# Nikhil-AI-Labs/image-super-resolution-2

Measured on AMD Instinct MI355X. Metric: output MPix/s at x4 SR (256->1024), higher is better.
Workload: dtype bf16 (bf16 MFMA operands, fp32 accumulate, fp32 activations in HBM); 1 GPU; FreqFusion x4 full 3-expert forward (HAT-L + DAT + NAFNet-SR + fusion stack), one 256x256 LR tile -> 1024x1024 per step per GPU (BASELINE configs[1]); seeded synthetic weights (172.3 M params), 1/f-noise tiles; tile=256, parallelism=tile-sharded x1, weights RCCL-broadcast once (0.0 ms), no per-tile collectives, launch=hipGraph replay, tiles_in_flight=2

## Files before the change

image-super-resolution-2_amd/csrc/token_linear.hip:

```cpp
#include "ff_common.h"


struct TokenLinParams {
  const float* x; float* out;
  const float* gamma; const float* beta;
  const __bf16* w;
  const float* bias;
  const float* res; const float* res2; const float* rs2;
  float* xn; int ldxn;
  float* stats; int st_lo, st_hi; float st_eps;
  const float* x2; int ldx2; const float* cm; const float* gw1t; const float* gb1; const float* gw2; float gb2;
  long long M;
  int ldx, ldo, ldr, ldr2, K, N, NT, act;
  float eps;
  int wpi;
};

#define TL_TR 36

#ifndef TL_GELU_SIG
#define TL_GELU_SIG 1
#endif
#define TL_KERNEL token_linear_kernel
#define TL_IMAGES 0
#define TL_OUT16 0
#include "token_linear_kernel.inc"
#undef TL_KERNEL
#undef TL_IMAGES
#define TL_KERNEL token_linear_images_kernel
#define TL_IMAGES 1
#include "token_linear_kernel.inc"
#undef TL_KERNEL
#undef TL_IMAGES
#undef TL_OUT16
#define TL_KERNEL token_linear_rows16_kernel
#define TL_IMAGES 0
#define TL_OUT16 1
#include "token_linear_kernel.inc"
#undef TL_KERNEL
#undef TL_IMAGES
#undef TL_OUT16


extern "C" int ff_token_linear(const float* x, int ldx, float* out, int ldo, long long M, int K, int kpad, int N, int n_tiles,
                               const float* gamma, const float* beta, float eps, const void* w_tiles,
                               const float* bias_padded, int act, const float* res, int ldr, const float* res2, int ldr2,
                               const float* res2_scale, float* xn_out, int ldxn, float* stats_out, int stat_lo, int stat_hi,
                               float stat_eps, int nterms, void* stream) {
  FF_CHECK_ARG(nterms == 1 || nterms == 3, "ff_token_linear: nterms must be 1 (plain bf16) or 3 (split bf16)");
  FF_CHECK_ARG(x && out && w_tiles, "ff_token_linear: null pointer");
  FF_CHECK_ARG(M > 0 && K > 0 && K <= 192 && K % 4 == 0 && N > 0 && n_tiles * 32 >= N, "ff_token_linear: needs K <= 192 (K %% 4 == 0), n_tiles*32 >= N");
  FF_CHECK_ARG(kpad == 64 || kpad == 128 || kpad == 192, "ff_token_linear: kpad must be 64, 128 or 192");
  FF_CHECK_ARG(kpad >= K, "ff_token_linear: kpad < K");
  FF_CHECK_ARG(ldx >= K && ldx % 4 == 0 && ldo >= N && (((uintptr_t)x) & 15) == 0, "ff_token_linear: x rows must be 16-byte aligned");
  FF_CHECK_ARG((gamma == nullptr) == (beta == nullptr), "ff_token_linear: gamma/beta come together");
  FF_CHECK_ARG((((uintptr_t)w_tiles) & 15) == 0 && (!gamma || ((((uintptr_t)gamma) & 15) == 0 && (((uintptr_t)beta) & 15) == 0)), "ff_token_linear: weights / gamma / beta must be 16-byte aligned");
  FF_CHECK_ARG(!res || ldr >= N, "ff_token_linear: ldr too small");
  FF_CHECK_ARG(!res2 || (ldr2 >= N && res2_scale), "ff_token_linear: res2 needs ldr2 >= N and a scale vector");
  FF_CHECK_ARG(!xn_out || (gamma && ldxn >= K && ldxn % 4 == 0 && (((uintptr_t)xn_out) & 15) == 0), "ff_token_linear: xn_out needs LayerNorm parameters and 16-byte aligned rows");
  TokenLinParams p;
  p.x = x; p.out = out; p.gamma = gamma; p.beta = beta; p.w = (const __bf16*)w_tiles; p.bias = bias_padded;
  p.res = res; p.res2 = res2; p.rs2 = res2_scale; p.xn = xn_out; p.ldxn = ldxn; p.M = M; p.ldx = ldx; p.ldo = ldo; p.ldr = ldr; p.ldr2 = ldr2;
  p.K = K; p.N = N; p.NT = n_tiles; p.act = act; p.eps = eps;
  FF_CHECK_ARG(!stats_out || (stat_lo >= 0 && stat_hi > stat_lo && stat_hi <= N && (((uintptr_t)stats_out) & 7) == 0), "ff_token_linear: bad statistics range");
  p.stats = stats_out; p.st_lo = stat_lo; p.st_hi = stat_hi; p.st_eps = stat_eps;
  p.x2 = nullptr; p.ldx2 = 0; p.cm = nullptr; p.gw1t = nullptr; p.gb1 = nullptr; p.gw2 = nullptr; p.gb2 = 0.f; p.wpi = 0;
  const bool vec4 = (N % 4 == 0) && (ldo % 4 == 0) && ((((uintptr_t)out) & 15) == 0) && (!res || (ldr % 4 == 0 && (((uintptr_t)res) & 15) == 0)) &&
           (!res2 || (ldr2 % 4 == 0 && (((uintptr_t)res2) & 15) == 0 && (((uintptr_t)res2_scale) & 15) == 0));
  const int ks = kpad / 16;
  const size_t lds = (size_t)2 * 2 * 32 * (2 * ks + 1) * 16 + (size_t)8 * 32 * TL_TR * 4 + (size_t)8 * 32 * FF_XS_ROW * 4 + (size_t)n_tiles * 32 * 4;
  FF_CHECK_ARG(lds <= 160 * 1024, "ff_token_linear: N too large for the LDS image");
  FF_CHECK_ARG(act == ACT_NONE || act == ACT_GELU, "ff_token_linear: act must be none or gelu");
  const long long nblk = (M + 255) / 256;
  FF_CHECK_ARG(nblk < (1LL << 31), "ff_token_linear: grid too large");
#define TL_LAUNCH(A, KSV, V4, NTM)                                                                                          \
  do {                                                                                                                      \
    static ff_device_once once;                                                                                             \
    if (!ff_raise_lds(once, "ff_token_linear", 160 * 1024, FF_LDS_SAY_ERR, &token_linear_kernel<A, KSV, V4, false, NTM>)) return FF_ERR_LAUNCH; \
    hipLaunchKernelGGL((token_linear_kernel<A, KSV, V4, false, NTM>), dim3((unsigned)nblk), dim3(512), lds, (hipStream_t)stream, p); \
  } while (0)
#define TL_LAUNCH_NT(A, KSV, V4) do { if (nterms == 3) TL_LAUNCH(A, KSV, V4, 3); else TL_LAUNCH(A, KSV, V4, 1); } while (0)
#define TL_LAUNCH_KS(A, V4) do { if (ks == 4) TL_LAUNCH_NT(A, 4, V4); else if (ks == 8) TL_LAUNCH_NT(A, 8, V4); else TL_LAUNCH_NT(A, 12, V4); } while (0)
  if (act == ACT_GELU) { if (vec4) TL_LAUNCH_KS(ACT_GELU, true); else TL_LAUNCH_KS(ACT_GELU, false); }
  else { if (vec4) TL_LAUNCH_KS(ACT_NONE, true); else TL_LAUNCH_KS(ACT_NONE, false); }
#undef TL_LAUNCH_KS
#undef TL_LAUNCH_NT
#undef TL_LAUNCH
  FF_LAUNCH_CHECK("ff_token_linear");
  return FF_OK;
}

extern "C" int ff_token_linear_rows16(const float* x, int ldx, void* out16, int ldo, long long M, int K, int kpad, int N, int n_tiles,
                                      const float* gamma, const float* beta, float eps, const void* w_tiles, const float* bias_padded,
                                      const float* col_scale, int act, const float* res, int ldr, const float* res2, int ldr2,
                                      const float* res2_scale, float* xn_out, int ldxn, float* stats_out, int stat_lo, int stat_hi,
                                      float stat_eps, int nterms, void* stream) {
  FF_CHECK_ARG(nterms == 1 && act == ACT_NONE && !res && !res2 && !res2_scale && !xn_out && !stats_out,
               "ff_token_linear_rows16: plain bf16 (nterms == 1), no activation, no res / res2 / xn_out / stats_out (got nterms=%d act=%d)", nterms, act);
  FF_CHECK_ARG(x && out16 && w_tiles && col_scale, "ff_token_linear_rows16: null pointer");
  FF_CHECK_ARG(M > 0 && K > 0 && K <= 192 && K % 4 == 0 && N > 0 && N % 4 == 0 && n_tiles * 32 >= N, "ff_token_linear_rows16: needs K <= 192, K and N multiples of 4, n_tiles*32 >= N");
  FF_CHECK_ARG(kpad == 64 || kpad == 128 || kpad == 192, "ff_token_linear_rows16: kpad must be 64, 128 or 192");
  FF_CHECK_ARG(kpad >= K, "ff_token_linear_rows16: kpad < K");
  FF_CHECK_ARG(ldx >= K && ldx % 4 == 0 && (((uintptr_t)x) & 15) == 0, "ff_token_linear_rows16: x rows must be 16-byte aligned");
  FF_CHECK_ARG(ldo >= N && ldo % 4 == 0 && (((uintptr_t)out16) & 7) == 0, "ff_token_linear_rows16: out rows must be 8-byte aligned (pitch in bf16 elements, a multiple of 4)");
  FF_CHECK_ARG((gamma == nullptr) == (beta == nullptr), "ff_token_linear_rows16: gamma/beta come together");
  FF_CHECK_ARG(((((uintptr_t)w_tiles) | ((uintptr_t)col_scale)) & 15) == 0 && (!gamma || ((((uintptr_t)gamma) & 15) == 0 && (((uintptr_t)beta) & 15) == 0)), "ff_token_linear_rows16: weights / col_scale / gamma / beta must be 16-byte aligned");
  TokenLinParams p;
  p.x = x; p.out = reinterpret_cast<float*>(out16); p.gamma = gamma; p.beta = beta; p.w = (const __bf16*)w_tiles; p.bias = bias_padded;
  p.res = nullptr; p.res2 = nullptr; p.rs2 = col_scale; p.xn = nullptr; p.ldxn = 0; p.M = M; p.ldx = ldx; p.ldo = ldo; p.ldr = 0; p.ldr2 = 0;
  p.K = K; p.N = N; p.NT = n_tiles; p.act = ACT_NONE; p.eps = eps;
  p.stats = nullptr; p.st_lo = 0; p.st_hi = 0; p.st_eps = 0.f;
  p.x2 = nullptr; p.ldx2 = 0; p.cm = nullptr; p.gw1t = nullptr; p.gb1 = nullptr; p.gw2 = nullptr; p.gb2 = 0.f; p.wpi = 0;
  const int ks = kpad / 16;
  const size_t lds = (size_t)2 * 2 * 32 * (2 * ks + 1) * 16 + (size_t)8 * 32 * TL_TR * 4 + (size_t)8 * 32 * FF_XS_ROW * 4 + (size_t)2 * n_tiles * 32 * 4;
  FF_CHECK_ARG(lds <= 160 * 1024, "ff_token_linear_rows16: N too large for the LDS image");
  const long long nblk = (M + 255) / 256;
  FF_CHECK_ARG(nblk < (1LL << 31), "ff_token_linear_rows16: grid too large");
#define TL_LAUNCH16(KSV)                                                                                                    \
  do {                                                                                                                      \
    static ff_device_once once;                                                                                             \
    if (!ff_raise_lds(once, "ff_token_linear_rows16", 160 * 1024, FF_LDS_SAY_ERR, &token_linear_rows16_kernel<ACT_NONE, KSV, true, false, 1>)) return FF_ERR_LAUNCH; \
    hipLaunchKernelGGL((token_linear_rows16_kernel<ACT_NONE, KSV, true, false, 1>), dim3((unsigned)nblk), dim3(512), lds, (hipStream_t)stream, p); \
  } while (0)
  if (ks == 4) TL_LAUNCH16(4); else if (ks == 8) TL_LAUNCH16(8); else TL_LAUNCH16(12);
#undef TL_LAUNCH16
  FF_LAUNCH_CHECK("ff_token_linear_rows16");
  return FF_OK;
}

static int token_linear_gated_launch(const char* who, const float* x, int ldx, const float* x2, int ldx2, const float* cm, int B, long long rows_per_image,
                                     const float* gw1t, const float* gb1, const float* gw2, float gb2, float* out, int ldo, long long M, int K, int N,
                                     int n_tiles, const void* w_tiles, const float* bias_padded, const float* res, int ldr, int nterms, void* stream) {
  FF_CHECK_ARG(nterms == 1 || nterms == 3, "%s: nterms must be 1 or 3", who);
  FF_CHECK_ARG(x && x2 && cm && gb1 && gw2 && out && w_tiles, "%s: null pointer", who);
  FF_CHECK_ARG(M > 0 && K > 0 && K <= 192 && K % 4 == 0 && N > 0 && N % 4 == 0 && n_tiles * 32 >= N, "%s: needs K <= 192, K and N multiples of 4", who);
  FF_CHECK_ARG(ldx >= K && ldx % 4 == 0 && ldx2 >= K && ldx2 % 4 == 0 && ldo >= N && ldo % 4 == 0 && (!res || (ldr >= N && ldr % 4 == 0)), "%s: rows must be 16-byte aligned", who);
  FF_CHECK_ARG(((((uintptr_t)x) | ((uintptr_t)x2) | ((uintptr_t)cm) | ((uintptr_t)out) | ((uintptr_t)w_tiles) | ((uintptr_t)res)) & 15) == 0, "%s: 16-byte alignment", who);
  const long long wpi = B ? rows_per_image / 256 : 0, nblk = B ? wpi : (M + 255) / 256;
  FF_CHECK_ARG(nblk < (1LL << 31), "%s: grid too large", who);
  TokenLinParams p{};
  p.x = x; p.out = out; p.w = (const __bf16*)w_tiles; p.bias = bias_padded; p.res = res; p.M = M; p.ldx = ldx; p.ldo = ldo; p.ldr = ldr;
  p.K = K; p.N = N; p.NT = n_tiles; p.act = ACT_NONE;
  p.x2 = x2; p.ldx2 = ldx2; p.cm = cm; p.gw1t = gw1t; p.gb1 = gb1; p.gw2 = gw2; p.gb2 = gb2; p.wpi = (int)wpi;
  const size_t lds = (size_t)2 * 2 * 32 * 25 * 16 + (size_t)8 * 32 * TL_TR * 4 + (size_t)8 * 32 * FF_XS_ROW * 4 + (size_t)n_tiles * 32 * 4;
  FF_CHECK_ARG(lds <= 160 * 1024, "%s: N too large for the LDS image", who);
  static ff_device_once once[2];
  if (!(!B ? ff_raise_lds(once[0], who, 160 * 1024, FF_LDS_SAY_ERR, &token_linear_kernel<ACT_NONE, 12, true, true, 3>, &token_linear_kernel<ACT_NONE, 12, true, true, 1>)
           : ff_raise_lds(once[1], who, 160 * 1024, FF_LDS_SAY_ERR, &token_linear_images_kernel<ACT_NONE, 12, true, true, 3>, &token_linear_images_kernel<ACT_NONE, 12, true, true, 1>)))
    return FF_ERR_LAUNCH;
  const dim3 grid((unsigned)nblk, B ? (unsigned)B : 1u);
  if (!B) {
    if (nterms == 3) hipLaunchKernelGGL((token_linear_kernel<ACT_NONE, 12, true, true, 3>), grid, dim3(512), lds, (hipStream_t)stream, p);
    else hipLaunchKernelGGL((token_linear_kernel<ACT_NONE, 12, true, true, 1>), grid, dim3(512), lds, (hipStream_t)stream, p);
  } else {
    if (nterms == 3) hipLaunchKernelGGL((token_linear_images_kernel<ACT_NONE, 12, true, true, 3>), grid, dim3(512), lds, (hipStream_t)stream, p);
    else hipLaunchKernelGGL((token_linear_images_kernel<ACT_NONE, 12, true, true, 1>), grid, dim3(512), lds, (hipStream_t)stream, p);
  }
  FF_LAUNCH_CHECK(who);
  return FF_OK;
}

extern "C" int ff_token_linear_gated(const float* x, int ldx, const float* x2, int ldx2, const float* cm, const float* gw1t,
                                     const float* gb1, const float* gw2, float gb2, float* out, int ldo, long long M, int K, int N,
                                     int n_tiles, const void* w_tiles, const float* bias_padded, const float* res, int ldr, int nterms,
                                     void* stream) {
  return token_linear_gated_launch("ff_token_linear_gated", x, ldx, x2, ldx2, cm, 0, 0, gw1t, gb1, gw2, gb2, out, ldo, M, K, N, n_tiles, w_tiles, bias_padded, res, ldr, nterms, stream);
}

extern "C" int ff_token_linear_gated_images(const float* x, int ldx, const float* x2, int ldx2, const float* cm, int B, long long rows_per_image,
                                            const float* gb1, const float* gw2, float gb2, float* out, int ldo, long long M, int K, int N,
                                            int n_tiles, const void* w_tiles, const float* bias_padded, const float* res, int ldr, int nterms,
                                            void* stream) {
  FF_CHECK_ARG(B > 0 && B <= 65535 && rows_per_image > 0 && rows_per_image % 256 == 0 && M == (long long)B * rows_per_image,
               "ff_token_linear_gated_images: rows_per_image must be a positive multiple of 256 and M == B * rows_per_image (1 <= B <= 65535; got B=%d rows_per_image=%lld M=%lld)",
               B, rows_per_image, M);
  return token_linear_gated_launch("ff_token_linear_gated_images", x, ldx, x2, ldx2, cm, B, rows_per_image, nullptr, gb1, gw2, gb2, out, ldo, M, K, N, n_tiles, w_tiles, bias_padded, res, ldr, nterms, stream);
}
```

image-super-resolution-2_amd/csrc/token_linear_kernel.inc:

```
template <int ACT, int TL_KS, bool VEC4, bool GATED = false, int NTERMS = 3>
__global__ __launch_bounds__(512) void TL_KERNEL(TokenLinParams p) {
  constexpr int TL_SLOTS = 2 * TL_KS + 1, TL_ROWB = TL_SLOTS * 16, TL_PL = 32 * TL_SLOTS, TL_PIECES = 2 * TL_PL / 64;
  constexpr int TL_TILE_ELEMS = 32 * 16 * TL_KS, KPAD = 16 * TL_KS;
  extern __shared__ __attribute__((aligned(16))) unsigned char smem[];
  constexpr int WB = TL_PL * 16;
  constexpr int BUFB = 2 * WB;
  const int tid = threadIdx.x, lane = tid & 63, wid = tid >> 6;
  const int l31 = lane & 31, hh = lane >> 5;
  float* tr = reinterpret_cast<float*>(smem + 2 * BUFB) + wid * (32 * TL_TR);
  float* xs = reinterpret_cast<float*>(smem + 2 * BUFB + 8 * 32 * TL_TR * 4) + wid * (32 * FF_XS_ROW);
  float* Bs = reinterpret_cast<float*>(smem + 2 * BUFB + 8 * 32 * TL_TR * 4 + 8 * 32 * FF_XS_ROW * 4);
#if TL_IMAGES
  const long long tok0 = ((long long)blockIdx.y * p.wpi + blockIdx.x) * 256 + wid * 32;
  const float* cmrow = p.cm + (long long)blockIdx.y * p.K;
#else
  const long long tok0 = (long long)blockIdx.x * 256 + wid * 32;
  const float* cmrow = p.cm;
#endif
  const long long tok = tok0 + l31;
  const bool tvalid = tok < p.M;

  int off[4];
#pragma unroll
  for (int i = 0; i < 4; ++i) {
    int s = (wid + 8 * i) * 64 + lane;
    if (s >= 2 * TL_PL) s = 2 * TL_PL - 1;
    const int plane = s / TL_PL, t = s - plane * TL_PL, row = t / TL_SLOTS;
    int q = t - row * TL_SLOTS;
    if (q > 2 * TL_KS - 1) q = 2 * TL_KS - 1;
    off[i] = plane * TL_TILE_ELEMS + row * KPAD + q * 8;
  }
  auto dma = [&](int nt, int buf) {
    const __bf16* rec = p.w + (long long)nt * (2 * TL_TILE_ELEMS);
#pragma unroll
    for (int i = 0; i < 4; ++i)
      if (wid + 8 * i < TL_PIECES)
        __builtin_amdgcn_global_load_lds((const __attribute__((address_space(1))) void*)(rec + off[i]),
                                         (__attribute__((address_space(3))) void*)(smem + buf * BUFB + (wid + 8 * i) * 1024), 16, 0, 0);
  };
  dma(0, 0);
  for (int i = tid; i < p.NT * 32; i += 512) Bs[i] = p.bias ? p.bias[i] : 0.f;
#if TL_OUT16
  float* Ss = Bs + p.NT * 32;
  for (int i = tid; i < p.NT * 32; i += 512) Ss[i] = p.rs2[i];
#endif

  bf16x8 xh[TL_KS], xl[TL_KS];
  if constexpr (GATED) {
    dma(p.NT, 1);
    float sm;
    {
      bf16x8 th[TL_KS], tl[TL_KS];
      {
        float v[TL_KS][8];
        ff_wave_rows_to_frags<TL_KS / 4>(p.x, p.ldx, tok0, p.M, p.K, xs, lane, v);
#pragma unroll
        for (int st = 0; st < TL_KS; ++st)
#pragma unroll
          for (int j = 0; j < 8; ++j) {
            const __bf16 h = (__bf16)v[st][j];
            th[st][j] = h;
            if (NTERMS == 3) tl[st][j] = (__bf16)(v[st][j] - (float)h);
          }
      }
      asm volatile("s_waitcnt vmcnt(0)" ::: "memory");
      __syncthreads();
      const unsigned char* ap = smem + BUFB + l31 * TL_ROWB + 16 * hh;
      f32x16 ga;
#pragma unroll
      for (int r = 0; r < 16; ++r) ga[r] = p.gb1[(r & 3) + 8 * (r >> 2) + 4 * hh];
      bf16x8 fa[2], fl[2];
#pragma unroll
      for (int u = 0; u < 2; ++u) {
        fa[u] = *reinterpret_cast<const bf16x8*>(ap + 32 * u);
        if (NTERMS == 3) fl[u] = *reinterpret_cast<const bf16x8*>(ap + 32 * u + WB);
      }
#pragma unroll
      for (int st = 0; st < TL_KS; ++st) {
        const bf16x8 ah = fa[st & 1], al = fl[st & 1];
        if (st + 2 < TL_KS) {
          fa[st & 1] = *reinterpret_cast<const bf16x8*>(ap + 32 * (st + 2));
          if (NTERMS == 3) fl[st & 1] = *reinterpret_cast<const bf16x8*>(ap + 32 * (st + 2) + WB);
        }
        __builtin_amdgcn_sched_barrier(0);
        if (NTERMS == 3) {
          ga = __builtin_amdgcn_mfma_f32_32x32x16_bf16(ah, tl[st], ga, 0, 0, 0);
          ga = __builtin_amdgcn_mfma_f32_32x32x16_bf16(al, th[st], ga, 0, 0, 0);
        }
        ga = __builtin_amdgcn_mfma_f32_32x32x16_bf16(ah, th[st], ga, 0, 0, 0);
        __builtin_amdgcn_sched_barrier(0);
      }
      float sacc = 0.f;
#pragma unroll
      for (int r = 0; r < 16; ++r) sacc += p.gw2[(r & 3) + 8 * (r >> 2) + 4 * hh] * ff_gelu_fast(ga[r]);
      sacc += __shfl_xor(sacc, 32);
      sm = 1.0f / (1.0f + expf(-(sacc + p.gb2)));
    }
    asm volatile("" ::: "memory");
    const int rr = lane >> 4, cq = (lane & 15) * 4;
#pragma unroll
    for (int pass = 0; pass < TL_KS / 4; ++pass) {
      asm volatile("" ::: "memory");
      f32x4 tS[8], tO[8];
#pragma unroll
      for (int j = 0; j < 8; ++j) {
        const int r = 4 * j + rr, c = 64 * pass + cq;
        const bool ok = tok0 + r < p.M && c < p.K;
        const f32x4 u = *reinterpret_cast<const f32x4*>(p.x + (ok ? (tok0 + r) * p.ldx + c : 0));
        const f32x4 w2 = *reinterpret_cast<const f32x4*>(p.x2 + (ok ? (tok0 + r) * p.ldx2 + c : 0));
        tS[j] = ok ? u : (f32x4){0.f, 0.f, 0.f, 0.f};
        tO[j] = ok ? w2 : (f32x4){0.f, 0.f, 0.f, 0.f};
      }
#pragma unroll
      for (int j = 0; j < 8; ++j) *reinterpret_cast<f32x4*>(xs + (4 * j + rr) * FF_XS_ROW + cq) = tS[j];
      f32x4 sa[4], sb[4];
#pragma unroll
      for (int s4 = 0; s4 < 4; ++s4) {
        sa[s4] = *reinterpret_cast<const f32x4*>(xs + l31 * FF_XS_ROW + 16 * s4 + 8 * hh);
        sb[s4] = *reinterpret_cast<const f32x4*>(xs + l31 * FF_XS_ROW + 16 * s4 + 8 * hh + 4);
      }
#pragma unroll
      for (int j = 0; j < 8; ++j) *reinterpret_cast<f32x4*>(xs + (4 * j + rr) * FF_XS_ROW + cq) = tO[j];
#pragma unroll
      for (int s4 = 0; s4 < 4; ++s4) {
        const int st = 4 * pass + s4, k0 = 16 * st + 8 * hh;
        const f32x4 oa = *reinterpret_cast<const f32x4*>(xs + l31 * FF_XS_ROW + 16 * s4 + 8 * hh);
        const f32x4 ob = *reinterpret_cast<const f32x4*>(xs + l31 * FF_XS_ROW + 16 * s4 + 8 * hh + 4);
        const int ka = k0 < p.K ? k0 : 0, kb = k0 + 4 < p.K ? k0 + 4 : 0;
        const f32x4 ca = *reinterpret_cast<const f32x4*>(cmrow + ka), cb = *reinterpret_cast<const f32x4*>(cmrow + kb);
        bf16x8 nh, nl;
#pragma unroll
        for (int j = 0; j < 8; ++j) {
          const float o = j < 4 ? oa[j & 3] : ob[j & 3], cmv = j < 4 ? ca[j & 3] : cb[j & 3];
          const float sv = j < 4 ? sa[s4][j & 3] : sb[s4][j & 3];
          const float f = (k0 + j < p.K) ? sv * cmv + o * sm : 0.f;
          const __bf16 h = (__bf16)f;
          nh[j] = h;
          if (NTERMS == 3) nl[j] = (__bf16)(f - (float)h);
        }
        xh[st] = nh;
        if (NTERMS == 3) {
          xl[st] = nl;
          asm volatile("" : "+v"(xh[st]), "+v"(xl[st]) : : "memory");
        } else {
          asm volatile("" : "+v"(xh[st]) : : "memory");
        }
      }
    }
  } else
  {
    float v[TL_KS][8];
    ff_wave_rows_to_frags<TL_KS / 4>(p.x, p.ldx, tok0, p.M, p.K, xs, lane, v);
    float mean = 0.f, rstd = 1.f;
    if (p.gamma) {
      float s = 0.f;
#pragma unroll
      for (int st = 0; st < TL_KS; ++st)
#pragma unroll
        for (int j = 0; j < 8; ++j) s += v[st][j];
      s += __shfl_xor(s, 32);
      mean = s / (float)p.K;
      float qv = 0.f;
#pragma unroll
      for (int st = 0; st < TL_KS; ++st)
#pragma unroll
        for (int j = 0; j < 8; ++j) {
          const float d = (16 * st + 8 * hh + j < p.K) ? v[st][j] - mean : 0.f;
          qv += d * d;
        }
      qv += __shfl_xor(qv, 32);
      rstd = 1.0f / sqrtf(qv / (float)p.K + p.eps);
    }
#pragma unroll
    for (int st = 0; st < TL_KS; ++st) {
      const int k0 = 16 * st + 8 * hh;
      f32x4 g0 = {1.f, 1.f, 1.f, 1.f}, g1 = g0, b0 = {0.f, 0.f, 0.f, 0.f}, b1 = b0;
      if (p.gamma) {
        const int ka = k0 < p.K ? k0 : 0, kb = k0 + 4 < p.K ? k0 + 4 : 0;
        g0 = *reinterpret_cast<const f32x4*>(p.gamma + ka); b0 = *reinterpret_cast<const f32x4*>(p.beta + ka);
        g1 = *reinterpret_cast<const f32x4*>(p.gamma + kb); b1 = *reinterpret_cast<const f32x4*>(p.beta + kb);
      }
#pragma unroll
      for (int j = 0; j < 8; ++j) {
        const float gg = j < 4 ? g0[j & 3] : g1[j & 3], bb = j < 4 ? b0[j & 3] : b1[j & 3];
        const float f = (k0 + j < p.K) ? (p.gamma ? (v[st][j] - mean) * rstd * gg + bb : v[st][j]) : 0.f;
        const __bf16 h = (__bf16)f;
        xh[st][j] = h;
        if (NTERMS == 3) xl[st][j] = (__bf16)(f - (float)h);
        v[st][j] = f;
      }
      if (p.xn && tvalid) {
        float* xr = p.xn + tok * p.ldxn + k0;
        if (k0 < p.K) *reinterpret_cast<f32x4*>(xr) = (f32x4){v[st][0], v[st][1], v[st][2], v[st][3]};
        if (k0 + 4 < p.K) *reinterpret_cast<f32x4*>(xr + 4) = (f32x4){v[st][4], v[st][5], v[st][6], v[st][7]};
      }
    }
  }

  float ssum = 0.f, ssq = 0.f;
  asm volatile("s_waitcnt vmcnt(0)" ::: "memory");
  for (int nt = 0; nt < p.NT; ++nt) {
    const int buf = nt & 1;
    asm volatile("s_waitcnt lgkmcnt(0)" ::: "memory");
    __builtin_amdgcn_s_barrier();
    if (nt + 1 < p.NT) dma(nt + 1, buf ^ 1);
    const int col = nt * 32 + l31;
    const bool cok = col < p.N;
    const int cc = cok ? col : 0;
    const int tq = lane >> 3, c4 = nt * 32 + 4 * (lane & 7);
    const bool c4ok = c4 < p.N;
    float rv[16];
    f32x4 rq[4];
    if (VEC4 && !TL_OUT16) {
#pragma unroll
      for (int i = 0; i < 4; ++i) {
        const long long tk = tok0 + tq + 8 * i;
        const bool ok = c4ok && tk < p.M;
        f32x4 r0 = {0.f, 0.f, 0.f, 0.f};
        if (p.res) { const f32x4 u = *reinterpret_cast<const f32x4*>(p.res + (ok ? tk * p.ldr + c4 : 0)); r0 = ok ? u : r0; }
        if (p.res2) {
          const f32x4 u = *reinterpret_cast<const f32x4*>(p.res2 + (ok ? tk * p.ldr2 + c4 : 0));
          const f32x4 sc = *reinterpret_cast<const f32x4*>(p.rs2 + (c4ok ? c4 : 0));
          if (ok) r0 += u * sc;
        }
        rq[i] = r0;
      }
    } else if (!VEC4) {
#pragma unroll
      for (int i = 0; i < 16; ++i) {
        const long long tk = tok0 + 2 * i + hh;
        const long long tqq = tk < p.M ? tk : 0;
        float r0 = p.res ? p.res[tqq * p.ldr + cc] : 0.f;
        if (p.res2) r0 += p.res2[tqq * p.ldr2 + cc] * p.rs2[cc];
        rv[i] = r0;
      }
    }
    const unsigned char* ap = smem + buf * BUFB + l31 * TL_ROWB + 16 * hh;
    f32x16 acc;
    {
      const int nb = nt * 32 + 4 * hh;
#pragma unroll
      for (int r = 0; r < 16; ++r) acc[r] = Bs[nb + (r & 3) + 8 * (r >> 2)];
    }
    bf16x8 fa[2], fl[2];
#pragma unroll
    for (int u = 0; u < 2; ++u) {
      fa[u] = *reinterpret_cast<const bf16x8*>(ap + 32 * u);
      if (NTERMS == 3) fl[u] = *reinterpret_cast<const bf16x8*>(ap + 32 * u + WB);
    }
#pragma unroll
    for (int st = 0; st < TL_KS; ++st) {
      const bf16x8 ah = fa[st & 1], al = fl[st & 1];
      if (st + 2 < TL_KS) {
        fa[st & 1] = *reinterpret_cast<const bf16x8*>(ap + 32 * (st + 2));
        if (NTERMS == 3) fl[st & 1] = *reinterpret_cast<const bf16x8*>(ap + 32 * (st + 2) + WB);
      }
      __builtin_amdgcn_sched_barrier(0);
      if (NTERMS == 3) {
        acc = __builtin_amdgcn_mfma_f32_32x32x16_bf16(ah, xl[st], acc, 0, 0, 0);
        acc = __builtin_amdgcn_mfma_f32_32x32x16_bf16(al, xh[st], acc, 0, 0, 0);
      }
      acc = __builtin_amdgcn_mfma_f32_32x32x16_bf16(ah, xh[st], acc, 0, 0, 0);
      __builtin_amdgcn_sched_barrier(0);
    }
#pragma unroll
    for (int g = 0; g < 4; ++g) {
      f32x4 v4;
      if (ACT == ACT_GELU && NTERMS == 1 && TL_GELU_SIG) {
        const f32x2 ga = ff_gelu_sig2((f32x2){acc[4 * g], acc[4 * g + 1]}), gb = ff_gelu_sig2((f32x2){acc[4 * g + 2], acc[4 * g + 3]});
        v4 = (f32x4){ga[0], ga[1], gb[0], gb[1]};
      } else {
#pragma unroll
        for (int e = 0; e < 4; ++e) v4[e] = ff_act_c<ACT, true>(acc[4 * g + e]);
      }
      *reinterpret_cast<f32x4*>(tr + l31 * TL_TR + 8 * g + 4 * hh) = v4;
      if (p.stats) {
        const int c0 = nt * 32 + 8 * g + 4 * hh;
#pragma unroll
        for (int e = 0; e < 4; ++e)
          if (c0 + e >= p.st_lo && c0 + e < p.st_hi) { ssum += v4[e]; ssq += v4[e] * v4[e]; }
      }
    }
    asm volatile("s_waitcnt vmcnt(0)" ::: "memory");
#if TL_OUT16
    {
      const f32x4 cs = *reinterpret_cast<const f32x4*>(Ss + nt * 32 + 4 * (lane & 7));
      bf16x4 ov[4];
#pragma unroll
      for (int i = 0; i < 4; ++i) {
        const f32x4 t4 = *reinterpret_cast<const f32x4*>(tr + (tq + 8 * i) * TL_TR + 4 * (lane & 7)) * cs;
        ov[i] = (bf16x4){(__bf16)t4[0], (__bf16)t4[1], (__bf16)t4[2], (__bf16)t4[3]};
      }
      if (c4ok) {
        __bf16* op = reinterpret_cast<__bf16*>(p.out) + (tok0 + tq) * p.ldo + c4;
        if (tok0 + 32 <= p.M) {
#pragma unroll
          for (int i = 0; i < 4; ++i) *reinterpret_cast<bf16x4*>(op + (long long)(8 * i) * p.ldo) = ov[i];
        } else {
#pragma unroll
          for (int i = 0; i < 4; ++i)
            if (tok0 + tq + 8 * i < p.M) *reinterpret_cast<bf16x4*>(op + (long long)(8 * i) * p.ldo) = ov[i];
        }
      }
    }
#else
    if (VEC4) {
      f32x4 ov[4];
#pragma unroll
      for (int i = 0; i < 4; ++i) ov[i] = *reinterpret_cast<const f32x4*>(tr + (tq + 8 * i) * TL_TR + 4 * (lane & 7)) + rq[i];
      if (c4ok) {
        float* op = p.out + (tok0 + tq) * p.ldo + c4;
        if (tok0 + 32 <= p.M) {
#pragma unroll
          for (int i = 0; i < 4; ++i) *reinterpret_cast<f32x4*>(op + (long long)(8 * i) * p.ldo) = ov[i];
        } else {
#pragma unroll
          for (int i = 0; i < 4; ++i)
            if (tok0 + tq + 8 * i < p.M) *reinterpret_cast<f32x4*>(op + (long long)(8 * i) * p.ldo) = ov[i];
        }
      }
    } else {
      float ov[16];
#pragma unroll
      for (int i = 0; i < 16; ++i) ov[i] = tr[(2 * i + hh) * TL_TR + l31] + rv[i];
      if (cok) {
        float* op = p.out + (tok0 + hh) * p.ldo + col;
        if (tok0 + 32 <= p.M) {
#pragma unroll
          for (int i = 0; i < 16; ++i) op[(long long)(2 * i) * p.ldo] = ov[i];
        } else {
#pragma unroll
          for (int i = 0; i < 16; ++i)
            if (tok0 + 2 * i + hh < p.M) op[(long long)(2 * i) * p.ldo] = ov[i];
        }
      }
    }
#endif
  }
  if (p.stats) {
    ssum += __shfl_xor(ssum, 32);
    ssq += __shfl_xor(ssq, 32);
    const float n = (float)(p.st_hi - p.st_lo);
    const float mean = ssum / n;
    const float var = fmaxf(ssq / n - mean * mean, 0.f);
    if (hh == 0 && tvalid) *reinterpret_cast<float2*>(p.stats + 2 * tok) = make_float2(mean, 1.0f / sqrtf(var + p.st_eps));
  }
}
```

Measured before the change: 27.61 output MPix/s.

## Triple-buffer weight DMA, stream residual via LDS DMA, use partial vmcnt waits

The token-linear kernel moves from double to triple buffering of the weight-tile DMA, prefetching two tiles ahead. The residual tile is now fetched into per-wave LDS with global_load_lds one n-tile ahead instead of with register loads issued inside the loop. The full vmcnt(0) drain before the epilogue becomes a computed partial wait, so in-flight prefetches and stores are not forced to finish. The LDS layout is reorganised to keep this within the limit: the transpose buffer and residual staging alias the xs rows, and the plane count is trimmed for nterms==1. The risk is fragile vmcnt accounting, where a wrong count would read stale data.

```diff
diff --git a/image-super-resolution-2_amd/csrc/token_linear.hip b/image-super-resolution-2_amd/csrc/token_linear.hip
--- a/image-super-resolution-2_amd/csrc/token_linear.hip
+++ b/image-super-resolution-2_amd/csrc/token_linear.hip
@@ -21,6 +21,20 @@
 #ifndef TL_GELU_SIG
 #define TL_GELU_SIG 1
 #endif
+
+__device__ __forceinline__ void tl_wait_vm(int n) {
+#define TL_VM(k) case k: asm volatile("s_waitcnt vmcnt(" #k ")" ::: "memory"); break;
+  switch (__builtin_amdgcn_readfirstlane(n)) {
+    TL_VM(1) TL_VM(2) TL_VM(3) TL_VM(4) TL_VM(5) TL_VM(6) TL_VM(7) TL_VM(8) TL_VM(16) TL_VM(17) TL_VM(18) TL_VM(19) TL_VM(20)
+    default: asm volatile("s_waitcnt vmcnt(0)" ::: "memory"); break;
+  }
+#undef TL_VM
+}
+
+static size_t tl_lds_bytes(int ks, int nterms, int n_tiles, int n_vec) {
+  const size_t pieces = ((size_t)(nterms == 3 ? 2 : 1) * 32 * (2 * ks + 1) + 63) / 64;
+  return 3 * pieces * 1024 + (size_t)8 * 32 * FF_XS_ROW * 4 + (size_t)n_vec * n_tiles * 32 * 4;
+}
 #define TL_KERNEL token_linear_kernel
 #define TL_IMAGES 0
 #define TL_OUT16 0
@@ -68,7 +82,7 @@
   const bool vec4 = (N % 4 == 0) && (ldo % 4 == 0) && ((((uintptr_t)out) & 15) == 0) && (!res || (ldr % 4 == 0 && (((uintptr_t)res) & 15) == 0)) &&
            (!res2 || (ldr2 % 4 == 0 && (((uintptr_t)res2) & 15) == 0 && (((uintptr_t)res2_scale) & 15) == 0));
   const int ks = kpad / 16;
-  const size_t lds = (size_t)2 * 2 * 32 * (2 * ks + 1) * 16 + (size_t)8 * 32 * TL_TR * 4 + (size_t)8 * 32 * FF_XS_ROW * 4 + (size_t)n_tiles * 32 * 4;
+  const size_t lds = tl_lds_bytes(ks, nterms, n_tiles, 1);
   FF_CHECK_ARG(lds <= 160 * 1024, "ff_token_linear: N too large for the LDS image");
   FF_CHECK_ARG(act == ACT_NONE || act == ACT_GELU, "ff_token_linear: act must be none or gelu");
   const long long nblk = (M + 255) / 256;
@@ -112,7 +126,7 @@
   p.stats = nullptr; p.st_lo = 0; p.st_hi = 0; p.st_eps = 0.f;
   p.x2 = nullptr; p.ldx2 = 0; p.cm = nullptr; p.gw1t = nullptr; p.gb1 = nullptr; p.gw2 = nullptr; p.gb2 = 0.f; p.wpi = 0;
   const int ks = kpad / 16;
-  const size_t lds = (size_t)2 * 2 * 32 * (2 * ks + 1) * 16 + (size_t)8 * 32 * TL_TR * 4 + (size_t)8 * 32 * FF_XS_ROW * 4 + (size_t)2 * n_tiles * 32 * 4;
+  const size_t lds = tl_lds_bytes(ks, 1, n_tiles, 2);
   FF_CHECK_ARG(lds <= 160 * 1024, "ff_token_linear_rows16: N too large for the LDS image");
   const long long nblk = (M + 255) / 256;
   FF_CHECK_ARG(nblk < (1LL << 31), "ff_token_linear_rows16: grid too large");
@@ -142,7 +156,7 @@
   p.x = x; p.out = out; p.w = (const __bf16*)w_tiles; p.bias = bias_padded; p.res = res; p.M = M; p.ldx = ldx; p.ldo = ldo; p.ldr = ldr;
   p.K = K; p.N = N; p.NT = n_tiles; p.act = ACT_NONE;
   p.x2 = x2; p.ldx2 = ldx2; p.cm = cm; p.gw1t = gw1t; p.gb1 = gb1; p.gw2 = gw2; p.gb2 = gb2; p.wpi = (int)wpi;
-  const size_t lds = (size_t)2 * 2 * 32 * 25 * 16 + (size_t)8 * 32 * TL_TR * 4 + (size_t)8 * 32 * FF_XS_ROW * 4 + (size_t)n_tiles * 32 * 4;
+  const size_t lds = tl_lds_bytes(12, nterms, n_tiles, 1);
   FF_CHECK_ARG(lds <= 160 * 1024, "%s: N too large for the LDS image", who);
   static ff_device_once once[2];
   if (!(!B ? ff_raise_lds(once[0], who, 160 * 1024, FF_LDS_SAY_ERR, &token_linear_kernel<ACT_NONE, 12, true, true, 3>, &token_linear_kernel<ACT_NONE, 12, true, true, 1>)
diff --git a/image-super-resolution-2_amd/csrc/token_linear_kernel.inc b/image-super-resolution-2_amd/csrc/token_linear_kernel.inc
--- a/image-super-resolution-2_amd/csrc/token_linear_kernel.inc
+++ b/image-super-resolution-2_amd/csrc/token_linear_kernel.inc
@@ -1,15 +1,20 @@
 template <int ACT, int TL_KS, bool VEC4, bool GATED = false, int NTERMS = 3>
 __global__ __launch_bounds__(512) void TL_KERNEL(TokenLinParams p) {
-  constexpr int TL_SLOTS = 2 * TL_KS + 1, TL_ROWB = TL_SLOTS * 16, TL_PL = 32 * TL_SLOTS, TL_PIECES = 2 * TL_PL / 64;
+  constexpr int TL_SLOTS = 2 * TL_KS + 1, TL_ROWB = TL_SLOTS * 16, TL_PL = 32 * TL_SLOTS;
+  constexpr int TL_NPL = NTERMS == 3 ? 2 : 1, TL_PIECES = (TL_NPL * TL_PL + 63) / 64;
   constexpr int TL_TILE_ELEMS = 32 * 16 * TL_KS, KPAD = 16 * TL_KS;
   extern __shared__ __attribute__((aligned(16))) unsigned char smem[];
   constexpr int WB = TL_PL * 16;
-  constexpr int BUFB = 2 * WB;
-  const int tid = threadIdx.x, lane = tid & 63, wid = tid >> 6;
+  constexpr int BUFB = TL_PIECES * 1024;
+  constexpr int TL_WPRIV = 32 * FF_XS_ROW * 4;
+  static_assert(32 * TL_TR * 4 + 32 * 32 * 4 <= TL_WPRIV && (32 * TL_TR * 4) % 16 == 0, "tr + rp must fit the wave's xs rows");
+  const int tid = threadIdx.x, lane = tid & 63, wid = __builtin_amdgcn_readfirstlane(tid >> 6);
   const int l31 = lane & 31, hh = lane >> 5;
-  float* tr = reinterpret_cast<float*>(smem + 2 * BUFB) + wid * (32 * TL_TR);
-  float* xs = reinterpret_cast<float*>(smem + 2 * BUFB + 8 * 32 * TL_TR * 4) + wid * (32 * FF_XS_ROW);
-  float* Bs = reinterpret_cast<float*>(smem + 2 * BUFB + 8 * 32 * TL_TR * 4 + 8 * 32 * FF_XS_ROW * 4);
+  unsigned char* wpriv = smem + 3 * BUFB + wid * TL_WPRIV;
+  float* xs = reinterpret_cast<float*>(wpriv);
+  float* tr = reinterpret_cast<float*>(wpriv);
+  unsigned char* rp = wpriv + 32 * TL_TR * 4;
+  float* Bs = reinterpret_cast<float*>(smem + 3 * BUFB + 8 * TL_WPRIV);
 #if TL_IMAGES
   const long long tok0 = ((long long)blockIdx.y * p.wpi + blockIdx.x) * 256 + wid * 32;
   const float* cmrow = p.cm + (long long)blockIdx.y * p.K;
@@ -24,7 +29,7 @@
 #pragma unroll
   for (int i = 0; i < 4; ++i) {
     int s = (wid + 8 * i) * 64 + lane;
-    if (s >= 2 * TL_PL) s = 2 * TL_PL - 1;
+    if (s >= TL_NPL * TL_PL) s = TL_NPL * TL_PL - 1;
     const int plane = s / TL_PL, t = s - plane * TL_PL, row = t / TL_SLOTS;
     int q = t - row * TL_SLOTS;
     if (q > 2 * TL_KS - 1) q = 2 * TL_KS - 1;
@@ -38,7 +43,9 @@
         __builtin_amdgcn_global_load_lds((const __attribute__((address_space(1))) void*)(rec + off[i]),
                                          (__attribute__((address_space(3))) void*)(smem + buf * BUFB + (wid + 8 * i) * 1024), 16, 0, 0);
   };
+  const int pw = wid < TL_PIECES ? (TL_PIECES - 1 - wid) / 8 + 1 : 0;
   dma(0, 0);
+  if (p.NT > 1) dma(1, 1);
   for (int i = tid; i < p.NT * 32; i += 512) Bs[i] = p.bias ? p.bias[i] : 0.f;
 #if TL_OUT16
   float* Ss = Bs + p.NT * 32;
@@ -47,7 +54,7 @@
 
   bf16x8 xh[TL_KS], xl[TL_KS];
   if constexpr (GATED) {
-    dma(p.NT, 1);
+    dma(p.NT, 2);
     float sm;
     {
       bf16x8 th[TL_KS], tl[TL_KS];
@@ -65,7 +72,7 @@
       }
       asm volatile("s_waitcnt vmcnt(0)" ::: "memory");
       __syncthreads();
-      const unsigned char* ap = smem + BUFB + l31 * TL_ROWB + 16 * hh;
+      const unsigned char* ap = smem + 2 * BUFB + l31 * TL_ROWB + 16 * hh;
       f32x16 ga;
 #pragma unroll
       for (int r = 0; r < 16; ++r) ga[r] = p.gb1[(r & 3) + 8 * (r >> 2) + 4 * hh];
@@ -198,34 +205,34 @@
   }
 
   float ssum = 0.f, ssq = 0.f;
-  asm volatile("s_waitcnt vmcnt(0)" ::: "memory");
+  const bool full = tok0 + 32 <= p.M;
+  constexpr int TL_NST = VEC4 ? 4 : 16;
+  const int tq = lane >> 3;
+  auto res_dma = [&](int nt) {
+    const int c4 = nt * 32 + 4 * (lane & 7);
+#pragma unroll
+    for (int i = 0; i < 4; ++i) {
+      const long long tk = tok0 + tq + 8 * i;
+      const bool ok = c4 < p.N && tk < p.M;
+      __builtin_amdgcn_global_load_lds((const __attribute__((address_space(1))) void*)(p.res + (ok ? tk * p.ldr + c4 : 0)),
+                                       (__attribute__((address_space(3))) void*)(rp + i * 1024), 16, 0, 0);
+    }
+  };
+  const bool res_lds = VEC4 && !TL_OUT16 && p.res != nullptr;
+  asm volatile("s_waitcnt vmcnt(0) lgkmcnt(0)" ::: "memory");
+  if (res_lds) res_dma(0);
   for (int nt = 0; nt < p.NT; ++nt) {
-    const int buf = nt & 1;
+    const int buf = nt % 3;
     asm volatile("s_waitcnt lgkmcnt(0)" ::: "memory");
     __builtin_amdgcn_s_barrier();
-    if (nt + 1 < p.NT) dma(nt + 1, buf ^ 1);
+    if (nt + 2 < p.NT) dma(nt + 2, (nt + 2) % 3);
     const int col = nt * 32 + l31;
     const bool cok = col < p.N;
     const int cc = cok ? col : 0;
-    const int tq = lane >> 3, c4 = nt * 32 + 4 * (lane & 7);
+    const int c4 = nt * 32 + 4 * (lane & 7);
     const bool c4ok = c4 < p.N;
     float rv[16];
-    f32x4 rq[4];
-    if (VEC4 && !TL_OUT16) {
-#pragma unroll
-      for (int i = 0; i < 4; ++i) {
-        const long long tk = tok0 + tq + 8 * i;
-        const bool ok = c4ok && tk < p.M;
-        f32x4 r0 = {0.f, 0.f, 0.f, 0.f};
-        if (p.res) { const f32x4 u = *reinterpret_cast<const f32x4*>(p.res + (ok ? tk * p.ldr + c4 : 0)); r0 = ok ? u : r0; }
-        if (p.res2) {
-          const f32x4 u = *reinterpret_cast<const f32x4*>(p.res2 + (ok ? tk * p.ldr2 + c4 : 0));
-          const f32x4 sc = *reinterpret_cast<const f32x4*>(p.rs2 + (c4ok ? c4 : 0));
-          if (ok) r0 += u * sc;
-        }
-        rq[i] = r0;
-      }
-    } else if (!VEC4) {
+    if (!VEC4) {
 #pragma unroll
       for (int i = 0; i < 16; ++i) {
         const long long tk = tok0 + 2 * i + hh;
@@ -281,7 +288,7 @@
           if (c0 + e >= p.st_lo && c0 + e < p.st_hi) { ssum += v4[e]; ssq += v4[e] * v4[e]; }
       }
     }
-    asm volatile("s_waitcnt vmcnt(0)" ::: "memory");
+    tl_wait_vm((nt + 2 < p.NT ? pw : 0) + (nt > 0 && full && (nt - 1) * 32 < p.N ? TL_NST : 0));
 #if TL_OUT16
     {
       const f32x4 cs = *reinterpret_cast<const f32x4*>(Ss + nt * 32 + 4 * (lane & 7));
@@ -305,9 +312,28 @@
     }
 #else
     if (VEC4) {
-      f32x4 ov[4];
-#pragma unroll
-      for (int i = 0; i < 4; ++i) ov[i] = *reinterpret_cast<const f32x4*>(tr + (tq + 8 * i) * TL_TR + 4 * (lane & 7)) + rq[i];
+      f32x4 ov[4], rq[4];
+#pragma unroll
+      for (int i = 0; i < 4; ++i) {
+        ov[i] = *reinterpret_cast<const f32x4*>(tr + (tq + 8 * i) * TL_TR + 4 * (lane & 7));
+        rq[i] = (f32x4){0.f, 0.f, 0.f, 0.f};
+        if (res_lds) rq[i] = *reinterpret_cast<const f32x4*>(rp + i * 1024 + lane * 16);
+      }
+      asm volatile("s_waitcnt lgkmcnt(0)" ::: "memory");
+      if (res_lds && nt + 1 < p.NT) res_dma(nt + 1);
+#pragma unroll
+      for (int i = 0; i < 4; ++i) {
+        const long long tk = tok0 + tq + 8 * i;
+        const bool ok = c4ok && tk < p.M;
+        f32x4 r0 = {0.f, 0.f, 0.f, 0.f};
+        if (p.res) r0 = ok ? rq[i] : r0;
+        if (p.res2) {
+          const f32x4 u = *reinterpret_cast<const f32x4*>(p.res2 + (ok ? tk * p.ldr2 + c4 : 0));
+          const f32x4 sc = *reinterpret_cast<const f32x4*>(p.rs2 + (c4ok ? c4 : 0));
+          if (ok) r0 += u * sc;
+        }
+        ov[i] += r0;
+      }
       if (c4ok) {
         float* op = p.out + (tok0 + tq) * p.ldo + c4;
         if (tok0 + 32 <= p.M) {
```

Measured after the change: 27.81 output MPix/s (median of 6 runs). Within noise of the previous version (+0.7%).
